# cts198859/deeprl_signal_control

Measured on AMD Instinct MI355X. Metric: env-steps/s (agents x envs x sim-steps/s), large_grid MA2C, higher is better.
Workload: dtype f32; 1 GPU; large_grid 5x5 (25 agents), MA2C LSTM policy (neighbour fingerprint gather), 1024 env instances per GPU; step = 120 control steps (x5 sim-steps) of every instance + 1 A2C update (BPTT, clip, RMSProp); envs_per_gpu=1024, n_step=120, agents=25, parallelism=env-sharded x1, live_vehicles=window mean over the timed region

## Files before the change

### deeprl_signal_control_amd/csrc/tsc_model.hip

```cpp
#include "tsc_common.h"
#include "tsc_gemm.h"
#include "../../include/tsc.h"

#include <cstdlib>
#include <type_traits>
#include <vector>

namespace {

using tsc::f32x16;
using tsc::f32x4;
using tsc::GemmArgs;

constexpr int kOut = 8;
constexpr int kL = 64;
constexpr int kG4 = 4 * kL;

struct Layout {
    int G, A, SMAX, AMAX, H;
    int NZ, fc;
    long long stride, oW1, ob1, oWx, oWh, obl, oWo, obo;
};

__device__ __forceinline__ float sigmoidf_(float x) {
// ... 102 lines not shown
            float keep = 1.0f;
            if (e < E) {
                const long long n = (long long)g * N + (long long)t * E + e;
                if (store) {
                    Z[n * kG4 + j] = ig; Z[n * kG4 + 64 + j] = fg; Z[n * kG4 + 128 + j] = og; Z[n * kG4 + 192 + j] = ug;
                    Cc[n * kL + j] = cn;
                }
                Hh[n * kL + j] = hn;
                if (t + 1 < T) keep = 1.0f - (float)done[(long long)(t + 1) * E + e];
                if (t + 1 == T && state_out) {
                    float *s = state_out + ((long long)g * E + e) * 2 * kL;
                    s[j] = cn; s[kL + j] = hn;
                }
            }
            c[r] = cn * keep;
            hs[j * kHsLd + erow[r]] = hn * keep;
        }
        __syncthreads();
    }
}

constexpr int kDz2Ld = kG4 + 4;
constexpr int kDh3Ld = kL + 4;

__global__ void __launch_bounds__(256, 2) lstm_bwd2_kernel(const float *__restrict__ params, Layout lay, float *Z,
                                                            const float *Cc, const float *state_bw, const float *dH,
                                                            const uint8_t *done, int T, int E) {
    extern __shared__ __attribute__((aligned(16))) char smem_raw[];
    float *dzs = (float *)smem_raw;
    float *dhs = dzs + 32 * kDz2Ld;
    const int g = blockIdx.x, e0 = blockIdx.y * 32;
    const int tid = threadIdx.x, lane = tid & 63, wave = tid >> 6, n = lane & 15, kq = lane >> 4;
    const int j = 16 * wave + n;
    const int er = tid >> 3, u0 = (tid & 7) * 8;
    const long long N = (long long)T * E;
    float bw[64];
    {
        const float4 *src = reinterpret_cast<const float4 *>(params + (long long)g * lay.stride + lay.oWh + (long long)j * kG4 + 4 * kq);
#pragma unroll
        for (int q = 0; q < 16; ++q) {
            const float4 w4 = src[4 * q];
            bw[4 * q] = w4.x; bw[4 * q + 1] = w4.y; bw[4 * q + 2] = w4.z; bw[4 * q + 3] = w4.w;
        }
    }
    float dc_rec[8];
#pragma unroll
    for (int r = 0; r < 8; ++r) dc_rec[r] = 0.f;
    const float *zg = Z + (long long)g * N * kG4, *cg = Cc + (long long)g * N * kL, *hg = dH + (long long)g * N * kL;
    const float *sg = state_bw + (long long)g * E * 2 * kL;
    const int e = e0 + er < E ? e0 + er : E - 1;
    const bool live = e0 + er < E;
    struct In { float4 gi[2], gf[2], go[2], gu[2], dhi[2], cpv[2]; float keep; };
    In in0, in1;
    float4 cc[2];
    auto request = [&](int t, In &o) {
        const long long nt = (long long)t * E;
        const float *zt = zg + nt * kG4, *ct = cg + nt * kL, *ht = hg + nt * kL;
        const float *cp_base = t > 0 ? ct - (long long)E * kL : sg;
        const unsigned cp_ld = t > 0 ? kL : 2 * kL;
        int zq = 0;
        asm volatile("" : "+v"(zq));
        const unsigned oz = (unsigned)((e + zq) * kG4 + u0) * 4u, oc = (unsigned)((e + zq) * kL + u0) * 4u;
#pragma unroll
        for (int a = 0; a < 2; ++a) {
            o.gi[a] = ldg((const float4 *)zt, oz + 16u * a); o.gf[a] = ldg((const float4 *)zt, oz + 256u + 16u * a);
            o.go[a] = ldg((const float4 *)zt, oz + 512u + 16u * a); o.gu[a] = ldg((const float4 *)zt, oz + 768u + 16u * a);
            o.dhi[a] = ldg((const float4 *)ht, oc + 16u * a);
            o.cpv[a] = ldg((const float4 *)cp_base, (unsigned)((e + zq) * cp_ld + u0) * 4u + 16u * a);
        }
        o.keep = done[nt + e] == 0 ? 1.0f : 0.0f;
    };
    {
        const float *ct = cg + (long long)(T - 1) * E * kL;
        cc[0] = ldg((const float4 *)ct, (unsigned)(e * kL + u0) * 4u); cc[1] = ldg((const float4 *)ct, (unsigned)(e * kL + u0) * 4u + 16u);
    }
    request(T - 1, in0);
    if (T > 1) request(T - 2, in1);
    float keep_next = 0.f;
    auto step = [&](int t, In &cur) {
        const long long nt = (long long)t * E;
        float *zw = Z + ((long long)g * N + nt) * kG4;
        const float keep = cur.keep;
        float4 dhr[2];
        if (t == T - 1) { dhr[0] = dhr[1] = make_float4(0.f, 0.f, 0.f, 0.f); }
        else {
            dhr[0] = *reinterpret_cast<const float4 *>(dhs + er * kDh3Ld + u0);
            dhr[1] = *reinterpret_cast<const float4 *>(dhs + er * kDh3Ld + u0 + 4);
        }
#pragma unroll
        for (int a = 0; a < 2; ++a) {
            const float igv[4] = {cur.gi[a].x, cur.gi[a].y, cur.gi[a].z, cur.gi[a].w}, fgv[4] = {cur.gf[a].x, cur.gf[a].y, cur.gf[a].z, cur.gf[a].w};
            const float ogv[4] = {cur.go[a].x, cur.go[a].y, cur.go[a].z, cur.go[a].w}, ugv[4] = {cur.gu[a].x, cur.gu[a].y, cur.gu[a].z, cur.gu[a].w};
            const float ccv[4] = {cc[a].x, cc[a].y, cc[a].z, cc[a].w}, cpw[4] = {cur.cpv[a].x, cur.cpv[a].y, cur.cpv[a].z, cur.cpv[a].w};
            const float dhv[4] = {cur.dhi[a].x, cur.dhi[a].y, cur.dhi[a].z, cur.dhi[a].w}, drv[4] = {dhr[a].x, dhr[a].y, dhr[a].z, dhr[a].w};
            float di[4], df[4], dg[4], du[4];
#pragma unroll
            for (int c = 0; c < 4; ++c) {
                const int r = 4 * a + c;
                const float ig = igv[c], fg = fgv[c], og = ogv[c], ug = ugv[c];
                const float cp = cpw[c] * keep;
                const float dh = dhv[c] + (keep_next != 0.f ? drv[c] : 0.f);
                const float tc = tanhf_(ccv[c]);
                dg[c] = dh * tc * og * (1.0f - og);
                const float dc = dh * og * (1.0f - tc * tc) + dc_rec[r];
                di[c] = dc * ug * ig * (1.0f - ig);
                df[c] = dc * cp * fg * (1.0f - fg);
                du[c] = dc * ig * (1.0f - ug * ug);
                dc_rec[r] = dc * fg * keep;
            }
            const float4 o_di = make_float4(di[0], di[1], di[2], di[3]), o_df = make_float4(df[0], df[1], df[2], df[3]);
            const float4 o_do = make_float4(dg[0], dg[1], dg[2], dg[3]), o_du = make_float4(du[0], du[1], du[2], du[3]);
            if (live) {
                const unsigned oz = (unsigned)((e0 + er) * kG4 + u0 + 4 * a) * 4u;
                stg((float4 *)zw, oz, o_di); stg((float4 *)zw, oz + 256u, o_df);
                stg((float4 *)zw, oz + 512u, o_do); stg((float4 *)zw, oz + 768u, o_du);
            }
            float *row = dzs + er * kDz2Ld + u0 + 4 * a;
// ... 3 lines not shown
        }
        cc[0] = cur.cpv[0]; cc[1] = cur.cpv[1];
        keep_next = keep;
        __syncthreads();
        if (t > 1) request(t - 2, cur);
        f32x4 acc[2];
        acc[0] = f32x4{0.f, 0.f, 0.f, 0.f}; acc[1] = f32x4{0.f, 0.f, 0.f, 0.f};
        const float4 *Aa = reinterpret_cast<const float4 *>(dzs + n * kDz2Ld + 4 * kq), *Ab = Aa + (16 * kDz2Ld) / 4;
        float4 pa = Aa[0], pb = Ab[0];
#pragma unroll
        for (int q = 0; q < 16; ++q) {
            const float4 na = Aa[4 * (q + 1 < 16 ? q + 1 : q)], nb = Ab[4 * (q + 1 < 16 ? q + 1 : q)];
            acc[0] = __builtin_amdgcn_mfma_f32_16x16x4f32(pa.x, bw[4 * q], acc[0], 0, 0, 0);
            acc[1] = __builtin_amdgcn_mfma_f32_16x16x4f32(pb.x, bw[4 * q], acc[1], 0, 0, 0);
            acc[0] = __builtin_amdgcn_mfma_f32_16x16x4f32(pa.y, bw[4 * q + 1], acc[0], 0, 0, 0);
            acc[1] = __builtin_amdgcn_mfma_f32_16x16x4f32(pb.y, bw[4 * q + 1], acc[1], 0, 0, 0);
            acc[0] = __builtin_amdgcn_mfma_f32_16x16x4f32(pa.z, bw[4 * q + 2], acc[0], 0, 0, 0);
            acc[1] = __builtin_amdgcn_mfma_f32_16x16x4f32(pb.z, bw[4 * q + 2], acc[1], 0, 0, 0);
            acc[0] = __builtin_amdgcn_mfma_f32_16x16x4f32(pa.w, bw[4 * q + 3], acc[0], 0, 0, 0);
            acc[1] = __builtin_amdgcn_mfma_f32_16x16x4f32(pb.w, bw[4 * q + 3], acc[1], 0, 0, 0);
            pa = na; pb = nb;
            __builtin_amdgcn_sched_barrier(0);
        }
#pragma unroll
        for (int rt = 0; rt < 2; ++rt)
#pragma unroll
            for (int i = 0; i < 4; ++i) dhs[(16 * rt + 4 * kq + i) * kDh3Ld + j] = acc[rt][i];
        __syncthreads();
    };
    for (int t = T - 1; t >= 0; t -= 2) {
        step(t, in0);
        if (t >= 1) step(t - 1, in1);
    }
}

__device__ __forceinline__ void head_eval(const float *__restrict__ params, const Layout &lay, int a, int na,
                                          const float *hp, const float *hv, float *pi, float &v) {
    const float *Wo = params + (long long)(2 * a) * lay.stride + lay.oWo;
    const float *bo = params + (long long)(2 * a) * lay.stride + lay.obo;
    const float *Wv = params + (long long)(2 * a + 1) * lay.stride + lay.oWo;
    const float *bv = params + (long long)(2 * a + 1) * lay.stride + lay.obo;
    float lg[kOut];
#pragma unroll
    for (int k = 0; k < kOut; ++k) lg[k] = 0.f;
    float vv = 0.f;
    for (int jj = 0; jj < kL; ++jj) {
        const float h = hp[jj];
#pragma unroll
        for (int k = 0; k < kOut; ++k) lg[k] += h * Wo[jj * kOut + k];
        vv += hv[jj] * Wv[jj * kOut];
    }
    float mx = -INFINITY;
#pragma unroll
    for (int k = 0; k < kOut; ++k) { lg[k] += bo[k]; if (k < na && lg[k] > mx) mx = lg[k]; }
    float sum = 0.f;
// ... 21 lines not shown
        if (r < rows_left)
            *reinterpret_cast<float4 *>(dst + (long long)r * kL + c) = make_float4(t[r][c], t[r][c + 1], t[r][c + 2], t[r][c + 3]);
    }
}

__global__ void __launch_bounds__(64) head_fwd_kernel(const float *__restrict__ params, Layout lay, const int *n_act,
                                                      const float *Hh, int E, float *pi_out, float *v_out) {
    __shared__ float sp[64][kTLd], sv[64][kTLd];
    const int a = blockIdx.y, lane = threadIdx.x;
    const long long n0 = (long long)blockIdx.x * 64, left = E - n0;
    tile_load(Hh + ((long long)(2 * a) * E + n0) * kL, left, sp, lane);
    tile_load(Hh + ((long long)(2 * a + 1) * E + n0) * kL, left, sv, lane);
    __syncthreads();
    if (lane >= left) return;
    float pi[kOut], v;
    head_eval(params, lay, a, n_act[a], sp[lane], sv[lane], pi, v);
    const long long idx = (n0 + lane) * lay.A + a;
    for (int k = 0; k < lay.AMAX; ++k) pi_out[idx * lay.AMAX + k] = k < kOut ? pi[k] : 0.f;
    v_out[idx] = v;
}

constexpr int kHbPer = kL * kOut + kOut + kL + 1;

__global__ void __launch_bounds__(256, 3)
head_bwd2_kernel(const float *__restrict__ params, Layout lay, const int *__restrict__ n_act, const float *__restrict__ Hh,
                 const int *__restrict__ act, const float *__restrict__ Rs, const float *__restrict__ Advs, long long N,
                 long long rows_per_slice, float v_coef, float beta, float *__restrict__ dH, float *__restrict__ part,
                 double *stats) {
    __shared__ float red[4][16][36];
    const int a = blockIdx.y, sp = blockIdx.x, na = n_act[a];
    const int tid = threadIdx.x, c = tid & 15, grp = tid >> 4;
    const float *Pp = params + (long long)(2 * a) * lay.stride, *Pv = params + (long long)(2 * a + 1) * lay.stride;
    float wo[4][kOut], wv[4], bo[kOut];
#pragma unroll
    for (int u = 0; u < 4; ++u) {
#pragma unroll
        for (int k = 0; k < kOut; ++k) wo[u][k] = Pp[lay.oWo + (4 * c + u) * kOut + k];
        wv[u] = Pv[lay.oWo + (4 * c + u) * kOut];
    }
#pragma unroll
    for (int k = 0; k < kOut; ++k) bo[k] = Pp[lay.obo + k];
    const float bv = Pv[lay.obo];
    float aw[4][kOut], awv[4], ab[kOut], abv = 0.f;
#pragma unroll
    for (int u = 0; u < 4; ++u) {
        awv[u] = 0.f;
#pragma unroll
        for (int k = 0; k < kOut; ++k) aw[u][k] = 0.f;
    }
#pragma unroll
    for (int k = 0; k < kOut; ++k) ab[k] = 0.f;
    float lp = 0.f, lv = 0.f, le = 0.f;
    const long long n0 = (long long)sp * rows_per_slice;
    long long n1 = n0 + rows_per_slice;
    if (n1 > N) n1 = N;
    const float *hp = Hh + (long long)(2 * a) * N * kL + 4 * c, *hq = Hh + (long long)(2 * a + 1) * N * kL + 4 * c;
    float *dp = dH + (long long)(2 * a) * N * kL + 4 * c, *dq = dH + (long long)(2 * a + 1) * N * kL + 4 * c;
    const float invN = 1.0f / (float)N;
    for (long long nb = n0; nb < n1; nb += 16) {
        const long long n = nb + grp;
        const bool in = n < n1;
        const long long nc = in ? n : n1 - 1;
        const float4 h4 = *reinterpret_cast<const float4 *>(hp + nc * kL);
        const float4 g4 = *reinterpret_cast<const float4 *>(hq + nc * kL);
        const long long idx = nc * lay.A + a;
        const int ac = act[idx];
        const float adv = Advs[idx], R = Rs[idx];
        const float hh[4] = {h4.x, h4.y, h4.z, h4.w}, gg[4] = {g4.x, g4.y, g4.z, g4.w};
        float lg[kOut], vv = 0.f;
#pragma unroll
        for (int k = 0; k < kOut; ++k) lg[k] = 0.f;
#pragma unroll
        for (int u = 0; u < 4; ++u) {
#pragma unroll
            for (int k = 0; k < kOut; ++k) lg[k] += hh[u] * wo[u][k];
            vv += gg[u] * wv[u];
        }
#pragma unroll
        for (int o = 1; o < 16; o <<= 1) {
#pragma unroll
// ... 22 lines not shown
            gpi += beta * invN * (logpm + (inr ? 1.0f : 0.f));
        }
        float dot = pim * gpi, ent = valid ? -pim * logpm : 0.f, lpa = (km == (ac < na ? ac : 0)) ? logpm : 0.f;
#pragma unroll
        for (int o = 1; o < 8; o <<= 1) {
            dot += __shfl_xor(dot, o, 64); ent += __shfl_xor(ent, o, 64); lpa += __shfl_xor(lpa, o, 64);
        }
        const float dlm = (in && valid) ? pim * (gpi - dot) : 0.f;
        float dl[kOut];
        const int row0 = (tid & 63) & ~15;
#pragma unroll
        for (int k = 0; k < kOut; ++k) dl[k] = __shfl(dlm, row0 + k, 64);
        const float dv = in ? v_coef * (v - R) * invN : 0.f;
        float o4[4], q4[4];
#pragma unroll
        for (int u = 0; u < 4; ++u) {
            float sacc = 0.f;
#pragma unroll
            for (int k = 0; k < kOut; ++k) { sacc += dl[k] * wo[u][k]; aw[u][k] += hh[u] * dl[k]; }
            o4[u] = (lay.fc && !(hh[u] > 0.f)) ? 0.f : sacc;
            q4[u] = (lay.fc && !(gg[u] > 0.f)) ? 0.f : dv * wv[u];
            awv[u] += gg[u] * dv;
        }
        if (in) {
            *reinterpret_cast<float4 *>(dp + n * kL) = make_float4(o4[0], o4[1], o4[2], o4[3]);
            *reinterpret_cast<float4 *>(dq + n * kL) = make_float4(q4[0], q4[1], q4[2], q4[3]);
        }
        if (c == 0) {
#pragma unroll
            for (int k = 0; k < kOut; ++k) ab[k] += dl[k];
            abv += dv;
            if (in) {
                lp += -lpa * adv * invN;
                lv += 0.5f * v_coef * (R - v) * (R - v) * invN;
                le += -beta * ent * invN;
            }
        }
    }
    const int wave = tid >> 6;
#pragma unroll
    for (int o = 16; o < 64; o <<= 1) {
#pragma unroll
        for (int u = 0; u < 4; ++u) {
#pragma unroll
            for (int k = 0; k < kOut; ++k) aw[u][k] += __shfl_xor(aw[u][k], o, 64);
            awv[u] += __shfl_xor(awv[u], o, 64);
        }
// ... 22 lines not shown
    float *out = part + ((long long)sp * lay.A + a) * kHbPer;
    for (int j = tid; j < kHbPer; j += 256) {
        float acc = 0.f;
        if (j < kL * kOut) {
            const int jj = j / kOut, k = j % kOut;
            for (int w = 0; w < 4; ++w) acc += red[w][jj >> 2][(jj & 3) * kOut + k];
        } else if (j < kL * kOut + kOut) {
            for (int w = 0; w < 4; ++w) acc += redb[w][j - kL * kOut];
        } else if (j < kL * kOut + kOut + kL) {
            const int jj = j - (kL * kOut + kOut);
            for (int w = 0; w < 4; ++w) acc += red[w][jj >> 2][32 + (jj & 3)];
        } else {
            for (int w = 0; w < 4; ++w) acc += redb[w][kOut];
        }
        out[j] = acc;
    }
    if (stats && tid == 0) {
        double a0 = 0, a1 = 0, a2 = 0;
        for (int w = 0; w < 4; ++w) { a0 += redl[w][0]; a1 += redl[w][1]; a2 += redl[w][2]; }
        atomicAdd(&stats[a * 4 + 0], a0); atomicAdd(&stats[a * 4 + 1], a1); atomicAdd(&stats[a * 4 + 2], a2);
    }
}

__global__ void __launch_bounds__(256, 3)
head_bwd_ppo_kernel(const float *__restrict__ params, Layout lay, const int *__restrict__ n_act, const float *__restrict__ Hh,
                    const int *__restrict__ act, const float *__restrict__ Rs, const float *__restrict__ Advs, long long N,
                    long long rows_per_slice, float v_coef, float beta, float *__restrict__ dH, float *__restrict__ part,
                    double *stats, float *__restrict__ logp_old, int record, float clip_eps, double *ppo_stats) {
    __shared__ float red[4][16][36];
    const int a = blockIdx.y, sp = blockIdx.x, na = n_act[a];
    const int tid = threadIdx.x, c = tid & 15, grp = tid >> 4;
    const float *Pp = params + (long long)(2 * a) * lay.stride, *Pv = params + (long long)(2 * a + 1) * lay.stride;
    float wo[4][kOut], wv[4], bo[kOut];
#pragma unroll
    for (int u = 0; u < 4; ++u) {
#pragma unroll
        for (int k = 0; k < kOut; ++k) wo[u][k] = Pp[lay.oWo + (4 * c + u) * kOut + k];
        wv[u] = Pv[lay.oWo + (4 * c + u) * kOut];
    }
#pragma unroll
    for (int k = 0; k < kOut; ++k) bo[k] = Pp[lay.obo + k];
    const float bv = Pv[lay.obo];
    float aw[4][kOut], awv[4], ab[kOut], abv = 0.f;
#pragma unroll
    for (int u = 0; u < 4; ++u) {
        awv[u] = 0.f;
#pragma unroll
        for (int k = 0; k < kOut; ++k) aw[u][k] = 0.f;
    }
#pragma unroll
    for (int k = 0; k < kOut; ++k) ab[k] = 0.f;
    float lp = 0.f, lv = 0.f, le = 0.f, lc = 0.f, lk = 0.f;
    const long long n0 = (long long)sp * rows_per_slice;
    long long n1 = n0 + rows_per_slice;
    if (n1 > N) n1 = N;
    const float *hp = Hh + (long long)(2 * a) * N * kL + 4 * c, *hq = Hh + (long long)(2 * a + 1) * N * kL + 4 * c;
    float *dp = dH + (long long)(2 * a) * N * kL + 4 * c, *dq = dH + (long long)(2 * a + 1) * N * kL + 4 * c;
    const float invN = 1.0f / (float)N;
    for (long long nb = n0; nb < n1; nb += 16) {
        const long long n = nb + grp;
        const bool in = n < n1;
        const long long nc = in ? n : n1 - 1;
        const float4 h4 = *reinterpret_cast<const float4 *>(hp + nc * kL);
        const float4 g4 = *reinterpret_cast<const float4 *>(hq + nc * kL);
        const long long idx = nc * lay.A + a;
        const int ac = act[idx];
        const float adv = Advs[idx], R = Rs[idx];
        const float hh[4] = {h4.x, h4.y, h4.z, h4.w}, gg[4] = {g4.x, g4.y, g4.z, g4.w};
        float lg[kOut], vv = 0.f;
#pragma unroll
        for (int k = 0; k < kOut; ++k) lg[k] = 0.f;
#pragma unroll
        for (int u = 0; u < 4; ++u) {
#pragma unroll
            for (int k = 0; k < kOut; ++k) lg[k] += hh[u] * wo[u][k];
            vv += gg[u] * wv[u];
        }
#pragma unroll
        for (int o = 1; o < 16; o <<= 1) {
#pragma unroll
// ... 29 lines not shown
            gpi += beta * invN * (logpm + (inr ? 1.0f : 0.f));
        }
        float dot = pim * gpi, ent = valid ? -pim * logpm : 0.f;
#pragma unroll
        for (int o = 1; o < 8; o <<= 1) {
            dot += __shfl_xor(dot, o, 64); ent += __shfl_xor(ent, o, 64);
        }
        const float dlm = (in && valid) ? pim * (gpi - dot) : 0.f;
        float dl[kOut];
        const int row0 = (tid & 63) & ~15;
#pragma unroll
        for (int k = 0; k < kOut; ++k) dl[k] = __shfl(dlm, row0 + k, 64);
        const float dv = in ? v_coef * (v - R) * invN : 0.f;
        float o4[4], q4[4];
#pragma unroll
        for (int u = 0; u < 4; ++u) {
            float sacc = 0.f;
#pragma unroll
            for (int k = 0; k < kOut; ++k) { sacc += dl[k] * wo[u][k]; aw[u][k] += hh[u] * dl[k]; }
            o4[u] = (lay.fc && !(hh[u] > 0.f)) ? 0.f : sacc;
            q4[u] = (lay.fc && !(gg[u] > 0.f)) ? 0.f : dv * wv[u];
            awv[u] += gg[u] * dv;
        }
        if (in) {
            *reinterpret_cast<float4 *>(dp + n * kL) = make_float4(o4[0], o4[1], o4[2], o4[3]);
            *reinterpret_cast<float4 *>(dq + n * kL) = make_float4(q4[0], q4[1], q4[2], q4[3]);
        }
        if (c == 0) {
#pragma unroll
            for (int k = 0; k < kOut; ++k) ab[k] += dl[k];
            abv += dv;
            if (in) {
                const float rc = fminf(fmaxf(ratio, 1.0f - clip_eps), 1.0f + clip_eps);
                lp += -fminf(ratio * adv, rc * adv) * invN;
                lc += clipped ? invN : 0.f;
                lk += (lpo - lpa) * invN;
                lv += 0.5f * v_coef * (R - v) * (R - v) * invN;
                le += -beta * ent * invN;
            }
        }
    }
    const int wave = tid >> 6;
#pragma unroll
    for (int o = 16; o < 64; o <<= 1) {
#pragma unroll
        for (int u = 0; u < 4; ++u) {
#pragma unroll
// ... 1664 lines not shown
}

namespace {

constexpr size_t kLdsMax = 160 * 1024;

template <int... W, class F> bool with_width(int H, F &&f) { return ((H == W && (f(std::integral_constant<int, W>{}), true)) || ...); }
template <class F> bool with_fused_width(int H, F &&f) { return with_width<128, 160, 192, 224>(H, f); }

enum class Fwd : int8_t {
    Dense,
    Tile,
    Ws,
    FcThread,
    FcMfma
};
inline bool fills_cache(Fwd f) { return f == Fwd::Tile || f == Fwd::Ws || f == Fwd::FcMfma; }

struct Plan {
    Fwd fwd;
    bool dwxh;
    bool dx1w1;
    bool fc_bwd;
    int s_fwd;
    int s_upd;
};

}

struct tsc_model {
    Layout lay;
    Plan plan;
    int E, T, device;
    double gamma, rnorm, rclip, vcoef, max_norm, alpha, eps;
    hipStream_t stream;
    tsc::DeviceBufs bufs;
    int *n_act;
    int16_t *rowrange;
    int *wgmap; unsigned fwd_wgs;
    int dbg_tid;
    int *ftmask;
    int *krange;
    float *params, *grads, *ms, *WxT;
    float *Wg;
    int wg_dirty;
    float *state_fw, *state_bw;
    float *r_obs; int *r_act; double *r_rew; float *r_val; uint8_t *r_done;
    float *Rs, *Advs;
    float *logp_old;
    int ppo_ready;
    float *X1, *Z, *Hh, *Cc, *Hp, *dHh;
    double *norm2, *stats, *norm_part;
    float *ws, *wsc;
    size_t ws_floats, wsc_floats;
    size_t lds_fwd, lds_fused, lds_ws;
    int inplace;
    int cached_next;
    long long *dbg;
    long long nparam;
};

namespace {

int gemm(tsc_model *m, int kid, bool tn, int epi, int groups, int M, int N, int K, const float *A, long long sA, int lda,
         int gdivA, const float *B, long long sB, int ldb, float *C, long long sC, int ldc, const float *bias,
         long long sBias, const float *aux, long long sAux, int ldaux, const int16_t *rr, long long sRR,
         float *colsum, long long sColsum) {
    GemmArgs a;
    a.A = A; a.B = B; a.C = C; a.bias = bias; a.aux = aux; a.rr = rr; a.colsum = colsum;
    a.sA = sA; a.sB = sB; a.sC = sC; a.sBias = sBias; a.sAux = sAux; a.sRR = sRR; a.sColsum = sColsum;
    a.lda = lda; a.ldb = ldb; a.ldc = ldc; a.ldaux = ldaux; a.M = M; a.N = N; a.K = K; a.gdivA = gdivA;
    tsc::plan_splitk(a, groups, tn ? m->ws : nullptr, m->wsc, m->ws_floats, m->wsc_floats);
    tsc::ProfScope ps(kid, m->stream);
    tsc::launch_gemm_dyn(tn, epi, a, groups, m->stream);
// ... 73 lines not shown
        std::vector<int> fm((size_t)L.A * ncu, 0);
        for (int a = 0; a < L.A; ++a)
            for (int u = 0; u < ncu; ++u)
                for (int j = 0; j < L.SMAX && j < 64; ++j) {
                    const int lo = rr[((size_t)a * L.SMAX + j) * 2], hi = rr[((size_t)a * L.SMAX + j) * 2 + 1];
                    if (lo < 16 * u + 16 && hi > 16 * u) fm[(size_t)a * ncu + u] |= 1 << (j >> 4);
                }
        TSC_HIP(m->bufs.upload(&m->ftmask, fm.data(), fm.size()));
    }
    TSC_HIP(m->bufs.upload(&m->n_act, cfg->n_act, L.A));
    const long long E = n_env, T = m->T, N = E * T, G = L.G, A = L.A;
    TSC_HIP(m->bufs.alloc(&m->params, m->nparam, true)); TSC_HIP(m->bufs.alloc(&m->grads, m->nparam, true)); TSC_HIP(m->bufs.alloc(&m->ms, m->nparam, true));
    TSC_HIP(m->bufs.alloc(&m->WxT, G * L.H * kG4, true));
    TSC_HIP(m->bufs.alloc(&m->Wg, G * (L.H + kL) * kG4, true));
    m->wg_dirty = 1;
    TSC_HIP(m->bufs.alloc(&m->state_fw, G * E * 2 * kL, true)); TSC_HIP(m->bufs.alloc(&m->state_bw, G * E * 2 * kL, true));
    TSC_HIP(m->bufs.alloc(&m->r_obs, (N + E) * A * L.SMAX, true));
    TSC_HIP(m->bufs.alloc(&m->r_act, N * A, true)); TSC_HIP(m->bufs.alloc(&m->r_rew, N * A, true));
    TSC_HIP(m->bufs.alloc(&m->r_val, N * A, true)); TSC_HIP(m->bufs.alloc(&m->r_done, (T + 1) * E, true));
    TSC_HIP(m->bufs.alloc(&m->Rs, N * A, true)); TSC_HIP(m->bufs.alloc(&m->Advs, N * A, true));
    TSC_HIP(m->bufs.alloc(&m->X1, G * N * L.H + 32 * L.H, true));
    TSC_HIP(m->bufs.alloc(&m->Z, G * N * kG4, true));
    TSC_HIP(m->bufs.alloc(&m->Hh, G * N * kL, true)); TSC_HIP(m->bufs.alloc(&m->Cc, G * N * kL, true)); TSC_HIP(m->bufs.alloc(&m->Hp, G * N * kL, true));
    TSC_HIP(m->bufs.alloc(&m->dHh, G * N * kL, true));
    TSC_HIP(m->bufs.alloc(&m->norm2, A, true)); TSC_HIP(m->bufs.alloc(&m->stats, A * 6, true));
    TSC_HIP(m->bufs.alloc(&m->norm_part, A * kNormParts, true));
    m->logp_old = nullptr; m->ppo_ready = 0;
    m->ws_floats = (size_t)48 << 20; m->wsc_floats = (size_t)1 << 20;
    TSC_HIP(m->bufs.alloc(&m->ws, m->ws_floats, true)); TSC_HIP(m->bufs.alloc(&m->wsc, m->wsc_floats, true));
    m->lds_fwd = sizeof(float) * (64 * kWhLd + 64 * kHsLd);
    m->lds_fused = sizeof(float) * ((size_t)(L.H + 64) * kXLd + kL * kOut + kOut + 8);
    m->lds_ws = sizeof(float) * ((size_t)32 * (L.H + 64 + 4) + 64 * kWsLdx + (size_t)kL * kWsLdg + (size_t)kG4 * kWsLdg + 528 + (kWsBuf + 2) * 32 * kOut + (size_t)L.SMAX * L.H);
    m->dbg = nullptr;
    m->cached_next = 0;
    m->inplace = 0;

    const auto env_int = [](const char *name, int unset) { const char *ev = getenv(name); return ev ? atoi(ev) : unset; };
    const char *fwd_ws = getenv("TSC_FWD_WS");
    const bool unfused_dx = env_int("TSC_UNFUSED_DX", 0) != 0;
    m->dbg_tid = env_int("TSC_DBG_THREAD", 0);
    Plan &P = m->plan;
    P.s_upd = 256 / (int)G;
    if (P.s_upd < 1) P.s_upd = 1;
    P.s_fwd = P.s_upd < (E + 31) / 32 ? P.s_upd : (int)((E + 31) / 32);
    const bool wide = with_fused_width(L.H, [](auto) {}), narrow_obs = L.SMAX <= 64;
    const auto ws_fits = [&](long long per_split) { return (size_t)(P.s_upd * G * per_split) <= m->ws_floats; };
    if (!L.fc) {
        const bool tile = L.H % 32 == 0 && narrow_obs && m->lds_fused <= kLdsMax;
        P.fwd = !tile ? Fwd::Dense : wide && m->lds_ws <= kLdsMax && !(fwd_ws && fwd_ws[0] == '0') ? Fwd::Ws : Fwd::Tile;
        size_t lds_dwxh = 0;
        with_fused_width(L.H, [&](auto w) { lds_dwxh = dwxh_lds<(decltype(w)::value + kL) / 32>(); });
        P.dwxh = wide && lds_dwxh <= kLdsMax && !env_int("TSC_UNFUSED_DW", 0) && ws_fits((long long)(L.H + kL + 1) * kG4);
        P.dx1w1 = wide && narrow_obs && !unfused_dx && ws_fits((long long)2 * 65 * L.H);
    } else {
        P.fwd = wide && narrow_obs && env_int("TSC_FC_MFMA", 1) ? Fwd::FcMfma
              : L.H % 16 == 0 && narrow_obs && fc_thread_lds(L.H) <= kLdsMax ? Fwd::FcThread : Fwd::Dense;
        P.fc_bwd = wide && narrow_obs && !unfused_dx && ws_fits((long long)2 * 65 * L.H + (long long)(L.H + 1) * kL);
    }
    m->fwd_wgs = (unsigned)(G * P.s_fwd);
    if (P.fwd == Fwd::Ws && env_int("TSC_FWD_XCD", 1) && P.s_fwd > 1 && P.s_fwd < 256) {
        const int S = P.s_fwd, cap = (L.G * S + 7) / 8;
        std::vector<int> tab((size_t)8 * cap, -1), used(8, 0);
        for (int gg = 0; gg < L.G; ++gg) {
            int left = S, spn = 0;
            while (left > 0) {
                int x = 0;
                for (int k = 1; k < 8; ++k) if (cap - used[k] > cap - used[x]) x = k;
                const int take = left < cap - used[x] ? left : cap - used[x];
                for (int q = 0; q < take; ++q) tab[(size_t)(used[x] + q) * 8 + x] = (gg << 8) | (spn + q);
                used[x] += take; spn += take; left -= take;
            }
        }
        TSC_HIP(m->bufs.upload(&m->wgmap, tab.data(), tab.size()));
        m->fwd_wgs = (unsigned)tab.size();
    }
    hipError_t attr = hipSuccess;
    const auto allow_lds = [&attr](const void *k) {
        if (attr == hipSuccess) attr = hipFuncSetAttribute(k, hipFuncAttributeMaxDynamicSharedMemorySize, (int)kLdsMax);
    };
    allow_lds((const void *)lstm_bwd2_kernel);
    allow_lds((const void *)lstm_fwd_kernel<true>);
    allow_lds((const void *)lstm_fwd_kernel<false>);
    if (P.fwd == Fwd::Tile) allow_lds((const void *)policy_fwd_fused_kernel);
    if (P.fwd == Fwd::FcThread) allow_lds((const void *)policy_fwd_fc_kernel);
    with_fused_width(L.H, [&](auto w) {
        constexpr int H = decltype(w)::value;
        if (P.fwd == Fwd::Ws) allow_lds((const void *)policy_fwd_ws_kernel<(H + kL) / 2>);
        if (P.fwd == Fwd::FcMfma) allow_lds((const void *)policy_fwd_fc_mfma_kernel<H / 32>);
        if (P.dwxh) allow_lds((const void *)dwxh_kernel<(H + kL) / 32>);
        if (P.dx1w1) allow_lds((const void *)dx1w1_kernel2<H / 16>);
        if (P.fc_bwd) allow_lds((const void *)fc_bwd_kernel<H / 16>);
    });
    TSC_HIP(attr);
    hipLaunchKernelGGL(fill_kernel, dim3((unsigned)((m->nparam + 255) / 256)), dim3(256), 0, 0, m->ms, m->nparam, 1.0f);
    TSC_HIP(hipDeviceSynchronize());
    *out = guard.release();
    return 0;
}

int tsc_model_destroy(tsc_model *m) {
    if (!m) return 0;
    (void)hipSetDevice(m->device);
    delete m;
// ... 187 lines not shown
    const Layout &L = m->lay;
    const long long E = m->E, A = L.A, no = E * A * L.SMAX;
    if (obs != m->r_obs + (size_t)t * no) m->inplace = 0;
    tsc::ProfScope ps5(tsc::KID_ADD_TRANS, m->stream);
    hipLaunchKernelGGL(add_transition_kernel, dim3((unsigned)((no + 255) / 256)), dim3(256), 0, m->stream, (int)E, (int)A,
                       L.SMAX, obs, done_pre, action, reward, value, done_post, m->r_obs + t * no,
                       m->r_act + t * E * A, m->r_rew + t * E * A, m->r_val + t * E * A, m->r_done + t * E,
                       m->r_done + (t + 1) * E);
    ps5.stop();
    TSC_HIP(hipGetLastError());
    return 0;
}

struct PpoArgs { double clip_eps, lambda; int epoch; };

static int launch_head_bwd(tsc_model *m, long long N, double beta, const PpoArgs *ppo) {
    const Layout &L = m->lay;
    hipStream_t st = m->stream;
    int S = (int)((8 * 256 + L.A - 1) / L.A);
    long long rps = (N + S - 1) / S;
    rps = (rps + 15) / 16 * 16;
    S = (int)((N + rps - 1) / rps);
    if ((size_t)((long long)S * L.A * kHbPer) > m->ws_floats) return tsc::fail("head_bwd: workspace too small");
    if (ppo) {
        tsc::ProfScope ps7(tsc::KID_HEAD_BWD_PPO, m->stream);
        hipLaunchKernelGGL(head_bwd_ppo_kernel, dim3((unsigned)S, (unsigned)L.A), dim3(256), 0, st, m->params, L, m->n_act, m->Hh, m->r_act,
                           m->Rs, m->Advs, N, rps, (float)m->vcoef, (float)beta, m->dHh, m->ws, m->stats, m->logp_old,
                           ppo->epoch == 0 ? 1 : 0, (float)ppo->clip_eps, m->stats + 4 * L.A);
    } else {
        tsc::ProfScope ps7(tsc::KID_HEAD_BWD, m->stream);
        hipLaunchKernelGGL(head_bwd2_kernel, dim3((unsigned)S, (unsigned)L.A), dim3(256), 0, st, m->params, L, m->n_act, m->Hh, m->r_act,
                           m->Rs, m->Advs, N, rps, (float)m->vcoef, (float)beta, m->dHh, m->ws, m->stats);
    }
    {
        tsc::ProfScope ps(tsc::KID_DWO_GEMM, m->stream);
        const int tot = L.A * 2 * (kL * kOut + kOut);
        hipLaunchKernelGGL(head_bwd2_reduce_kernel, dim3((tot + 255) / 256), dim3(256), 0, st, m->ws, L.A, S, m->grads, L);
    }
    return hipGetLastError() == hipSuccess ? 0 : 1;
}

int tsc_model_rollout_slot(tsc_model *m, int32_t t, void *ptrs[6]) {
    if (!m || !ptrs || t < 0 || t > m->T) return tsc::fail("tsc_model_rollout_slot: slot %d outside [0,%d]", t, m ? m->T : 0);
    const Layout &L = m->lay;
    const long long E = m->E, A = L.A, no = E * A * L.SMAX;
    const bool in = t < m->T;
    ptrs[0] = m->r_obs + t * no;
    ptrs[1] = in ? (void *)(m->r_act + t * E * A) : nullptr;
    ptrs[2] = in ? (void *)(m->r_val + t * E * A) : nullptr;
    ptrs[3] = in ? (void *)(m->r_rew + t * E * A) : nullptr;
    ptrs[4] = m->r_done + t * E;
    ptrs[5] = in ? (void *)(m->r_done + (t + 1) * E) : nullptr;
    return 0;
}

// ... 36 lines not shown
                tsc::ProfScope ps(tsc::KID_DW1_GEMM, m->stream);
                const long long tot = ((long long)(L.SMAX + 1) * L.H + (long long)(L.H + 1) * kL) * G;
                hipLaunchKernelGGL(fc_bwd_reduce_kernel, dim3((unsigned)((tot + 255) / 256)), dim3(256), 0, st, m->ws, (int)G, S, L.H, L.SMAX,
                                   m->rowrange, g, L.stride, L.oW1, L.ob1, L.oWx);
            }
            TSC_HIP(hipGetLastError());
            m->cached_next = 0;
            return 0;
        }
        if (gemm(m, tsc::KID_DWX_GEMM, true, tsc::EPI_NONE, (int)G, L.H, kL, (int)N, m->X1, N * L.H, L.H, 1, m->dHh, N * kL, kL, g + L.oWx,
                 L.stride, kL, nullptr, 0, nullptr, 0, 0, nullptr, 0, g + L.obl, L.stride)) return tsc::fail("gemm failed");
        if (gemm(m, tsc::KID_DX1_GEMM, false, tsc::EPI_MASK_POS, (int)G, (int)N, L.H, kL, m->dHh, N * kL, kL, 1, m->WxT, (long long)L.H * kL, L.H,
                 m->X1, N * L.H, L.H, nullptr, 0, m->X1, N * L.H, L.H, nullptr, 0, nullptr, 0)) return tsc::fail("gemm failed");
    } else {
    if (m->cached_next != (int)T) {
        if (dense_forward(m, m->r_obs, N, m->X1, m->Z)) return tsc::fail("gemm launch failed");
        tsc::ProfScope ps2(tsc::KID_LSTM_FWD, m->stream);
        hipLaunchKernelGGL(lstm_fwd_kernel<true>, dim3((unsigned)G, (unsigned)((E + 63) / 64)), dim3(256), m->lds_fwd, st, m->params, L,
                           m->Z, m->state_bw, (float *)nullptr, m->Hh, m->Cc, m->Hp, m->r_done, (int)T, (int)E, 1);
        ps2.stop();
    }
    if (launch_head_bwd(m, N, beta, ppo)) return tsc::fail("head_bwd failed");
    tsc::ProfScope ps8(tsc::KID_LSTM_BWD, m->stream);
    hipLaunchKernelGGL(lstm_bwd2_kernel, dim3((unsigned)G, (unsigned)((E + 31) / 32)), dim3(256), sizeof(float) * 32 * (kDz2Ld + kDh3Ld), st,
                       m->params, L, m->Z, m->Cc, m->state_bw, m->dHh, m->r_done, (int)T, (int)E);
    ps8.stop();
    tsc::ProfScope ps9(tsc::KID_TRANSPOSE, m->stream);
    hipLaunchKernelGGL(transpose_wx_kernel, dim3((unsigned)((G * L.H * kG4 + 255) / 256)), dim3(256), 0, st, m->params, L, m->WxT);
    ps9.stop();
    TSC_HIP(hipGetLastError());
    if (P.dwxh) {
        const long long per = (long long)(L.H + kL + 1) * kG4;
        long long rps = (N + S - 1) / S;
        rps += rps & 1;
        {
            tsc::ProfScope ps(tsc::KID_DWX_GEMM, m->stream);
            with_fused_width(L.H, [&](auto w) {
                constexpr int NT = (decltype(w)::value + kL) / 32;
                hipLaunchKernelGGL(dwxh_kernel<NT>, dim3((unsigned)(S * G)), dim3(512), dwxh_lds<NT>(), st, m->X1, m->Hp, m->Z, N, (int)G, S,
                                   rps, m->ws, m->dbg);
            });
        }
        {
            tsc::ProfScope ps(tsc::KID_DWH_GEMM, m->stream);
            hipLaunchKernelGGL(dwxh_reduce_kernel, dim3((unsigned)((per * G + 255) / 256)), dim3(256), 0, st, m->ws, (int)G, S, per, g,
                               L.stride, L.oWx);
        }
        TSC_HIP(hipGetLastError());
// ... 127 lines not shown
    if (!m || !Rs || !Advs) return tsc::fail("tsc_model_get_returns: bad arguments");
    const size_t n = (size_t)m->T * m->E * m->lay.A;
    TSC_HIP(hipStreamSynchronize(m->stream));
    TSC_HIP(hipMemcpy(Rs, m->Rs, sizeof(float) * n, hipMemcpyDeviceToHost));
    TSC_HIP(hipMemcpy(Advs, m->Advs, sizeof(float) * n, hipMemcpyDeviceToHost));
    return 0;
}

int tsc_model_debug_read(tsc_model *m, int32_t what, int32_t g, int64_t row0, int64_t nrows, float *out_host) {
    if (!m || !out_host || g < 0 || g >= m->lay.G || row0 < 0 || nrows < 0) return tsc::fail("tsc_model_debug_read: bad arguments");
    const long long N = (long long)m->T * m->E;
    if (row0 + nrows > N) return tsc::fail("tsc_model_debug_read: rows [%lld, %lld) outside [0, %lld)", (long long)row0, (long long)(row0 + nrows), N);
    const float *base = nullptr;
    long long w = 0;
    switch (what) {
        case 0: base = m->X1; w = m->lay.H; break;
        case 1: base = m->Z; w = kG4; break;
        case 2: base = m->Hh; w = kL; break;
        case 3: base = m->Cc; w = kL; break;
        case 4: base = m->Hp; w = kL; break;
        case 5: base = m->dHh; w = kL; break;
        default: return tsc::fail("tsc_model_debug_read: unknown buffer %d", what);
    }
    if (m->lay.fc && (what == 1 || what == 3 || what == 4)) return tsc::fail("tsc_model_debug_read: buffer %d is LSTM-only", what);
    TSC_HIP(hipStreamSynchronize(m->stream));
    TSC_HIP(hipMemcpy(out_host, base + ((long long)g * N + row0) * w, sizeof(float) * (size_t)(nrows * w), hipMemcpyDeviceToHost));
    return 0;
}

int tsc_gemm_grouped_f32(int32_t form, int32_t epi, int32_t groups, int32_t M, int32_t N, int32_t K, const float *A,
                         int64_t sA, int32_t lda, const float *B, int64_t sB, int32_t ldb, float *C, int64_t sC,
                         int32_t ldc, const float *bias, const float *aux, const int16_t *rowrange, float *colsum,
                         float *splitk_ws, int64_t ws_floats, float *splitk_wsc, int64_t wsc_floats, void *hip_stream) {
    GemmArgs a;
    a.A = A; a.B = B; a.C = C; a.bias = bias; a.aux = aux; a.rr = rowrange; a.colsum = colsum;
    a.sA = sA; a.sB = sB; a.sC = sC; a.sBias = N; a.sAux = (long long)M * ldc; a.sRR = M; a.sColsum = N;
    a.lda = lda; a.ldb = ldb; a.ldc = ldc; a.ldaux = ldc; a.M = M; a.N = N; a.K = K; a.gdivA = 1;
    tsc::plan_splitk(a, groups, form != 0 ? splitk_ws : nullptr, splitk_wsc, (size_t)ws_floats, (size_t)wsc_floats);
    tsc::launch_gemm_dyn(form != 0, epi, a, groups, (hipStream_t)hip_stream);
    TSC_HIP(hipGetLastError());
    return 0;
}

}
```

Before: 397.5 million env-steps/s.

## Pass compact logit/value gradients to LSTM backward instead of full dH

The head backward kernels now write per-row logit gradients (8 floats) and a scalar value gradient instead of 64-wide dH vectors for the policy and value LSTMs. The LSTM backward kernel loads Wo into LDS and rebuilds dh on the fly: an 8x8 dot per row for the policy group, and a scalar times a weight column for the value group. This cuts dH write and read traffic roughly eightfold and shrinks its buffer, at the cost of extra ALU and LDS reads in the BPTT loop. The old path stays available through an environment flag.

```diff
diff --git a/deeprl_signal_control_amd/csrc/tsc_model.hip b/deeprl_signal_control_amd/csrc/tsc_model.hip
--- a/deeprl_signal_control_amd/csrc/tsc_model.hip
+++ b/deeprl_signal_control_amd/csrc/tsc_model.hip
@@ -148,13 +148,17 @@
 
 constexpr int kDz2Ld = kG4 + 4;
 constexpr int kDh3Ld = kL + 4;
-
+constexpr int kWoLd = 8 * kOut + 4;
+constexpr size_t lstm_bwd2_lds(bool rec) { return sizeof(float) * (32 * (kDz2Ld + kDh3Ld) + (rec ? 8 * kWoLd : 0)); }
+
+template <bool kRec>
 __global__ void __launch_bounds__(256, 2) lstm_bwd2_kernel(const float *__restrict__ params, Layout lay, float *Z,
                                                             const float *Cc, const float *state_bw, const float *dH,
-                                                            const uint8_t *done, int T, int E) {
+                                                            const float *DV, const uint8_t *done, int T, int E) {
     extern __shared__ __attribute__((aligned(16))) char smem_raw[];
     float *dzs = (float *)smem_raw;
     float *dhs = dzs + 32 * kDz2Ld;
+    float *wos = dhs + 32 * kDh3Ld;
     const int g = blockIdx.x, e0 = blockIdx.y * 32;
     const int tid = threadIdx.x, lane = tid & 63, wave = tid >> 6, n = lane & 15, kq = lane >> 4;
     const int j = 16 * wave + n;
@@ -172,16 +176,26 @@
     float dc_rec[8];
 #pragma unroll
     for (int r = 0; r < 8; ++r) dc_rec[r] = 0.f;
-    const float *zg = Z + (long long)g * N * kG4, *cg = Cc + (long long)g * N * kL, *hg = dH + (long long)g * N * kL;
+    const bool pol = (g & 1) == 0;
+    if constexpr (kRec) {
+        const float *src = params + (long long)g * lay.stride + lay.oWo;
+        if (pol) { for (int i = tid; i < kL * kOut; i += 256) wos[(i >> 6) * kWoLd + (i & 63)] = src[i]; }
+        else if (tid < kL) wos[(tid >> 3) * kWoLd + (tid & 7)] = src[tid * kOut];
+        __syncthreads();
+    }
+    const float *wo = wos + (tid & 7) * kWoLd;
+    const float *zg = Z + (long long)g * N * kG4, *cg = Cc + (long long)g * N * kL;
+    const float *hg = kRec ? dH + (long long)(g >> 1) * N * kOut : dH + (long long)g * N * kL;
+    const float *vg = kRec ? DV + (long long)(g >> 1) * N : nullptr;
     const float *sg = state_bw + (long long)g * E * 2 * kL;
     const int e = e0 + er < E ? e0 + er : E - 1;
     const bool live = e0 + er < E;
-    struct In { float4 gi[2], gf[2], go[2], gu[2], dhi[2], cpv[2]; float keep; };
+    struct In { float4 gi[2], gf[2], go[2], gu[2], hd[2], cpv[2]; float keep; };
     In in0, in1;
     float4 cc[2];
     auto request = [&](int t, In &o) {
         const long long nt = (long long)t * E;
-        const float *zt = zg + nt * kG4, *ct = cg + nt * kL, *ht = hg + nt * kL;
+        const float *zt = zg + nt * kG4, *ct = cg + nt * kL, *ht = hg + nt * (kRec ? kOut : kL);
         const float *cp_base = t > 0 ? ct - (long long)E * kL : sg;
         const unsigned cp_ld = t > 0 ? kL : 2 * kL;
         int zq = 0;
@@ -191,10 +205,39 @@
         for (int a = 0; a < 2; ++a) {
             o.gi[a] = ldg((const float4 *)zt, oz + 16u * a); o.gf[a] = ldg((const float4 *)zt, oz + 256u + 16u * a);
             o.go[a] = ldg((const float4 *)zt, oz + 512u + 16u * a); o.gu[a] = ldg((const float4 *)zt, oz + 768u + 16u * a);
-            o.dhi[a] = ldg((const float4 *)ht, oc + 16u * a);
+            if constexpr (!kRec) o.hd[a] = ldg((const float4 *)ht, oc + 16u * a);
             o.cpv[a] = ldg((const float4 *)cp_base, (unsigned)((e + zq) * cp_ld + u0) * 4u + 16u * a);
         }
+        if constexpr (kRec) {
+            if (pol) {
+                o.hd[0] = ldg((const float4 *)ht, (unsigned)((e + zq) * kOut) * 4u);
+                o.hd[1] = ldg((const float4 *)ht, (unsigned)((e + zq) * kOut) * 4u + 16u);
+            } else {
+                o.hd[0].x = ldg(vg + nt, (unsigned)(e + zq) * 4u);
+            }
+        }
         o.keep = done[nt + e] == 0 ? 1.0f : 0.0f;
+    };
+    auto expand = [&](In &o) {
+        float d[8];
+        if (pol) {
+            const float dl[kOut] = {o.hd[0].x, o.hd[0].y, o.hd[0].z, o.hd[0].w, o.hd[1].x, o.hd[1].y, o.hd[1].z, o.hd[1].w};
+#pragma unroll
+            for (int r = 0; r < 8; ++r) {
+                const float4 lo = *reinterpret_cast<const float4 *>(wo + 8 * r), hi = *reinterpret_cast<const float4 *>(wo + 8 * r + 4);
+                const float w[kOut] = {lo.x, lo.y, lo.z, lo.w, hi.x, hi.y, hi.z, hi.w};
+                float sacc = 0.f;
+#pragma unroll
+                for (int k = 0; k < kOut; ++k) sacc += dl[k] * w[k];
+                d[r] = sacc;
+            }
+        } else {
+            const float4 lo = *reinterpret_cast<const float4 *>(wo), hi = *reinterpret_cast<const float4 *>(wo + 4);
+            const float dv = o.hd[0].x;
+            d[0] = dv * lo.x; d[1] = dv * lo.y; d[2] = dv * lo.z; d[3] = dv * lo.w;
+            d[4] = dv * hi.x; d[5] = dv * hi.y; d[6] = dv * hi.z; d[7] = dv * hi.w;
+        }
+        o.hd[0] = make_float4(d[0], d[1], d[2], d[3]); o.hd[1] = make_float4(d[4], d[5], d[6], d[7]);
     };
     {
         const float *ct = cg + (long long)(T - 1) * E * kL;
@@ -202,8 +245,9 @@
     }
     request(T - 1, in0);
     if (T > 1) request(T - 2, in1);
+    if constexpr (kRec) expand(in0);
     float keep_next = 0.f;
-    auto step = [&](int t, In &cur) {
+    auto step = [&](int t, In &cur, In &nxt) {
         const long long nt = (long long)t * E;
         float *zw = Z + ((long long)g * N + nt) * kG4;
         const float keep = cur.keep;
@@ -218,7 +262,8 @@
             const float igv[4] = {cur.gi[a].x, cur.gi[a].y, cur.gi[a].z, cur.gi[a].w}, fgv[4] = {cur.gf[a].x, cur.gf[a].y, cur.gf[a].z, cur.gf[a].w};
             const float ogv[4] = {cur.go[a].x, cur.go[a].y, cur.go[a].z, cur.go[a].w}, ugv[4] = {cur.gu[a].x, cur.gu[a].y, cur.gu[a].z, cur.gu[a].w};
             const float ccv[4] = {cc[a].x, cc[a].y, cc[a].z, cc[a].w}, cpw[4] = {cur.cpv[a].x, cur.cpv[a].y, cur.cpv[a].z, cur.cpv[a].w};
-            const float dhv[4] = {cur.dhi[a].x, cur.dhi[a].y, cur.dhi[a].z, cur.dhi[a].w}, drv[4] = {dhr[a].x, dhr[a].y, dhr[a].z, dhr[a].w};
+            const float drv[4] = {dhr[a].x, dhr[a].y, dhr[a].z, dhr[a].w};
+            const float dhv[4] = {cur.hd[a].x, cur.hd[a].y, cur.hd[a].z, cur.hd[a].w};
             float di[4], df[4], dg[4], du[4];
 #pragma unroll
             for (int c = 0; c < 4; ++c) {
@@ -268,6 +313,7 @@
             pa = na; pb = nb;
             __builtin_amdgcn_sched_barrier(0);
         }
+        if constexpr (kRec) { if (t > 0) expand(nxt); }
 #pragma unroll
         for (int rt = 0; rt < 2; ++rt)
 #pragma unroll
@@ -275,8 +321,8 @@
         __syncthreads();
     };
     for (int t = T - 1; t >= 0; t -= 2) {
-        step(t, in0);
-        if (t >= 1) step(t - 1, in1);
+        step(t, in0, in1);
+        if (t >= 1) step(t - 1, in1, in0);
     }
 }
 
@@ -344,11 +390,12 @@
 
 constexpr int kHbPer = kL * kOut + kOut + kL + 1;
 
+template <bool kRec>
 __global__ void __launch_bounds__(256, 3)
 head_bwd2_kernel(const float *__restrict__ params, Layout lay, const int *__restrict__ n_act, const float *__restrict__ Hh,
                  const int *__restrict__ act, const float *__restrict__ Rs, const float *__restrict__ Advs, long long N,
-                 long long rows_per_slice, float v_coef, float beta, float *__restrict__ dH, float *__restrict__ part,
-                 double *stats) {
+                 long long rows_per_slice, float v_coef, float beta, float *__restrict__ dH, float *__restrict__ DV,
+                 float *__restrict__ part, double *stats) {
     __shared__ float red[4][16][36];
     const int a = blockIdx.y, sp = blockIdx.x, na = n_act[a];
     const int tid = threadIdx.x, c = tid & 15, grp = tid >> 4;
@@ -377,7 +424,8 @@
     long long n1 = n0 + rows_per_slice;
     if (n1 > N) n1 = N;
     const float *hp = Hh + (long long)(2 * a) * N * kL + 4 * c, *hq = Hh + (long long)(2 * a + 1) * N * kL + 4 * c;
-    float *dp = dH + (long long)(2 * a) * N * kL + 4 * c, *dq = dH + (long long)(2 * a + 1) * N * kL + 4 * c;
+    float *dp = kRec ? dH + (long long)a * N * kOut + (c & 7) : dH + (long long)(2 * a) * N * kL + 4 * c;
+    float *dq = kRec ? DV + (long long)a * N : dH + (long long)(2 * a + 1) * N * kL + 4 * c;
     const float invN = 1.0f / (float)N;
     for (long long nb = n0; nb < n1; nb += 16) {
         const long long n = nb + grp;
@@ -446,7 +494,10 @@
             q4[u] = (lay.fc && !(gg[u] > 0.f)) ? 0.f : dv * wv[u];
             awv[u] += gg[u] * dv;
         }
-        if (in) {
+        if constexpr (kRec) {
+            if (in && c < 8) dp[n * kOut] = dlm;
+            if (in && c == 8) dq[n] = dv;
+        } else if (in) {
             *reinterpret_cast<float4 *>(dp + n * kL) = make_float4(o4[0], o4[1], o4[2], o4[3]);
             *reinterpret_cast<float4 *>(dq + n * kL) = make_float4(q4[0], q4[1], q4[2], q4[3]);
         }
@@ -515,11 +566,12 @@
     }
 }
 
+template <bool kRec>
 __global__ void __launch_bounds__(256, 3)
 head_bwd_ppo_kernel(const float *__restrict__ params, Layout lay, const int *__restrict__ n_act, const float *__restrict__ Hh,
                     const int *__restrict__ act, const float *__restrict__ Rs, const float *__restrict__ Advs, long long N,
-                    long long rows_per_slice, float v_coef, float beta, float *__restrict__ dH, float *__restrict__ part,
-                    double *stats, float *__restrict__ logp_old, int record, float clip_eps, double *ppo_stats) {
+                    long long rows_per_slice, float v_coef, float beta, float *__restrict__ dH, float *__restrict__ DV,
+                    float *__restrict__ part, double *stats, float *__restrict__ logp_old, int record, float clip_eps, double *ppo_stats) {
     __shared__ float red[4][16][36];
     const int a = blockIdx.y, sp = blockIdx.x, na = n_act[a];
     const int tid = threadIdx.x, c = tid & 15, grp = tid >> 4;
@@ -548,7 +600,8 @@
     long long n1 = n0 + rows_per_slice;
     if (n1 > N) n1 = N;
     const float *hp = Hh + (long long)(2 * a) * N * kL + 4 * c, *hq = Hh + (long long)(2 * a + 1) * N * kL + 4 * c;
-    float *dp = dH + (long long)(2 * a) * N * kL + 4 * c, *dq = dH + (long long)(2 * a + 1) * N * kL + 4 * c;
+    float *dp = kRec ? dH + (long long)a * N * kOut + (c & 7) : dH + (long long)(2 * a) * N * kL + 4 * c;
+    float *dq = kRec ? DV + (long long)a * N : dH + (long long)(2 * a + 1) * N * kL + 4 * c;
     const float invN = 1.0f / (float)N;
     for (long long nb = n0; nb < n1; nb += 16) {
         const long long n = nb + grp;
@@ -624,7 +677,10 @@
             q4[u] = (lay.fc && !(gg[u] > 0.f)) ? 0.f : dv * wv[u];
             awv[u] += gg[u] * dv;
         }
-        if (in) {
+        if constexpr (kRec) {
+            if (in && c < 8) dp[n * kOut] = dlm;
+            if (in && c == 8) dq[n] = dv;
+        } else if (in) {
             *reinterpret_cast<float4 *>(dp + n * kL) = make_float4(o4[0], o4[1], o4[2], o4[3]);
             *reinterpret_cast<float4 *>(dq + n * kL) = make_float4(q4[0], q4[1], q4[2], q4[3]);
         }
@@ -2335,6 +2391,7 @@
     bool dwxh;
     bool dx1w1;
     bool fc_bwd;
+    bool head_dl;
     int s_fwd;
     int s_upd;
 };
@@ -2362,7 +2419,9 @@
     float *Rs, *Advs;
     float *logp_old;
     int ppo_ready;
-    float *X1, *Z, *Hh, *Cc, *Hp, *dHh;
+    float *X1, *Z, *Hh, *Cc, *Hp;
+    float *dHh;
+    float *DL, *DV;
     double *norm2, *stats, *norm_part;
     float *ws, *wsc;
     size_t ws_floats, wsc_floats;
@@ -2482,7 +2541,6 @@
     TSC_HIP(m->bufs.alloc(&m->X1, G * N * L.H + 32 * L.H, true));
     TSC_HIP(m->bufs.alloc(&m->Z, G * N * kG4, true));
     TSC_HIP(m->bufs.alloc(&m->Hh, G * N * kL, true)); TSC_HIP(m->bufs.alloc(&m->Cc, G * N * kL, true)); TSC_HIP(m->bufs.alloc(&m->Hp, G * N * kL, true));
-    TSC_HIP(m->bufs.alloc(&m->dHh, G * N * kL, true));
     TSC_HIP(m->bufs.alloc(&m->norm2, A, true)); TSC_HIP(m->bufs.alloc(&m->stats, A * 6, true));
     TSC_HIP(m->bufs.alloc(&m->norm_part, A * kNormParts, true));
     m->logp_old = nullptr; m->ppo_ready = 0;
@@ -2512,11 +2570,14 @@
         with_fused_width(L.H, [&](auto w) { lds_dwxh = dwxh_lds<(decltype(w)::value + kL) / 32>(); });
         P.dwxh = wide && lds_dwxh <= kLdsMax && !env_int("TSC_UNFUSED_DW", 0) && ws_fits((long long)(L.H + kL + 1) * kG4);
         P.dx1w1 = wide && narrow_obs && !unfused_dx && ws_fits((long long)2 * 65 * L.H);
+        P.head_dl = !env_int("TSC_HEAD_DH", 0);
     } else {
         P.fwd = wide && narrow_obs && env_int("TSC_FC_MFMA", 1) ? Fwd::FcMfma
               : L.H % 16 == 0 && narrow_obs && fc_thread_lds(L.H) <= kLdsMax ? Fwd::FcThread : Fwd::Dense;
         P.fc_bwd = wide && narrow_obs && !unfused_dx && ws_fits((long long)2 * 65 * L.H + (long long)(L.H + 1) * kL);
     }
+    if (P.head_dl) { TSC_HIP(m->bufs.alloc(&m->DL, A * N * kOut, true)); TSC_HIP(m->bufs.alloc(&m->DV, A * N, true)); }
+    else { TSC_HIP(m->bufs.alloc(&m->dHh, G * N * kL, true)); }
     m->fwd_wgs = (unsigned)(G * P.s_fwd);
     if (P.fwd == Fwd::Ws && env_int("TSC_FWD_XCD", 1) && P.s_fwd > 1 && P.s_fwd < 256) {
         const int S = P.s_fwd, cap = (L.G * S + 7) / 8;
@@ -2538,7 +2599,7 @@
     const auto allow_lds = [&attr](const void *k) {
         if (attr == hipSuccess) attr = hipFuncSetAttribute(k, hipFuncAttributeMaxDynamicSharedMemorySize, (int)kLdsMax);
     };
-    allow_lds((const void *)lstm_bwd2_kernel);
+    if (!L.fc) allow_lds(P.head_dl ? (const void *)lstm_bwd2_kernel<true> : (const void *)lstm_bwd2_kernel<false>);
     allow_lds((const void *)lstm_fwd_kernel<true>);
     allow_lds((const void *)lstm_fwd_kernel<false>);
     if (P.fwd == Fwd::Tile) allow_lds((const void *)policy_fwd_fused_kernel);
@@ -2772,15 +2833,18 @@
     rps = (rps + 15) / 16 * 16;
     S = (int)((N + rps - 1) / rps);
     if ((size_t)((long long)S * L.A * kHbPer) > m->ws_floats) return tsc::fail("head_bwd: workspace too small");
+    const bool rec = m->plan.head_dl;
+    float *hd = rec ? m->DL : m->dHh;
     if (ppo) {
         tsc::ProfScope ps7(tsc::KID_HEAD_BWD_PPO, m->stream);
-        hipLaunchKernelGGL(head_bwd_ppo_kernel, dim3((unsigned)S, (unsigned)L.A), dim3(256), 0, st, m->params, L, m->n_act, m->Hh, m->r_act,
-                           m->Rs, m->Advs, N, rps, (float)m->vcoef, (float)beta, m->dHh, m->ws, m->stats, m->logp_old,
-                           ppo->epoch == 0 ? 1 : 0, (float)ppo->clip_eps, m->stats + 4 * L.A);
+        hipLaunchKernelGGL(rec ? head_bwd_ppo_kernel<true> : head_bwd_ppo_kernel<false>, dim3((unsigned)S, (unsigned)L.A), dim3(256), 0, st,
+                           m->params, L, m->n_act, m->Hh, m->r_act, m->Rs, m->Advs, N, rps, (float)m->vcoef, (float)beta, hd, m->DV, m->ws,
+                           m->stats, m->logp_old, ppo->epoch == 0 ? 1 : 0, (float)ppo->clip_eps, m->stats + 4 * L.A);
     } else {
         tsc::ProfScope ps7(tsc::KID_HEAD_BWD, m->stream);
-        hipLaunchKernelGGL(head_bwd2_kernel, dim3((unsigned)S, (unsigned)L.A), dim3(256), 0, st, m->params, L, m->n_act, m->Hh, m->r_act,
-                           m->Rs, m->Advs, N, rps, (float)m->vcoef, (float)beta, m->dHh, m->ws, m->stats);
+        hipLaunchKernelGGL(rec ? head_bwd2_kernel<true> : head_bwd2_kernel<false>, dim3((unsigned)S, (unsigned)L.A), dim3(256), 0, st,
+                           m->params, L, m->n_act, m->Hh, m->r_act, m->Rs, m->Advs, N, rps, (float)m->vcoef, (float)beta, hd, m->DV, m->ws,
+                           m->stats);
     }
     {
         tsc::ProfScope ps(tsc::KID_DWO_GEMM, m->stream);
@@ -2863,8 +2927,9 @@
     }
     if (launch_head_bwd(m, N, beta, ppo)) return tsc::fail("head_bwd failed");
     tsc::ProfScope ps8(tsc::KID_LSTM_BWD, m->stream);
-    hipLaunchKernelGGL(lstm_bwd2_kernel, dim3((unsigned)G, (unsigned)((E + 31) / 32)), dim3(256), sizeof(float) * 32 * (kDz2Ld + kDh3Ld), st,
-                       m->params, L, m->Z, m->Cc, m->state_bw, m->dHh, m->r_done, (int)T, (int)E);
+    hipLaunchKernelGGL(P.head_dl ? lstm_bwd2_kernel<true> : lstm_bwd2_kernel<false>, dim3((unsigned)G, (unsigned)((E + 31) / 32)), dim3(256),
+                       lstm_bwd2_lds(P.head_dl), st, m->params, L, m->Z, m->Cc, m->state_bw, P.head_dl ? m->DL : m->dHh, m->DV,
+                       m->r_done, (int)T, (int)E);
     ps8.stop();
     tsc::ProfScope ps9(tsc::KID_TRANSPOSE, m->stream);
     hipLaunchKernelGGL(transpose_wx_kernel, dim3((unsigned)((G * L.H * kG4 + 255) / 256)), dim3(256), 0, st, m->params, L, m->WxT);
@@ -3038,6 +3103,9 @@
         case 5: base = m->dHh; w = kL; break;
         default: return tsc::fail("tsc_model_debug_read: unknown buffer %d", what);
     }
+    if (what == 5 && !base)
+        return tsc::fail("tsc_model_debug_read: buffer 5 (dH) does not exist on this handle: its head pass hands BPTT logit-gradient "
+                         "records instead (TSC_HEAD_DH=1 at create keeps dH)");
     if (m->lay.fc && (what == 1 || what == 3 || what == 4)) return tsc::fail("tsc_model_debug_read: buffer %d is LSTM-only", what);
     TSC_HIP(hipStreamSynchronize(m->stream));
     TSC_HIP(hipMemcpy(out_host, base + ((long long)g * N + row0) * w, sizeof(float) * (size_t)(nrows * w), hipMemcpyDeviceToHost));
```

Result: no change. 397.7 million env-steps/s (median of 3 runs) (+0.1%).
